# batra-mlp-lab/visdial

Hardware: AMD Instinct MI355X
Metric: QA-rounds/sec training mn-att-ques-im-hist+disc (batch 20x10x100) (higher is better)
Workload: dtype f32 operands and results; the option recurrence multiplies the EXACT 3-way bf16 split of both operands (9 bf16 MFMA products per fp32 product, f32 accumulate: fp32-grade, errors at the f32 MFMA's own level) -- its two step kernels and its weight-gradient contraction; f32 MFMA (v_mfma_f32_32x32x2_f32

## Files before the change

### visdial_amd/csrc/split_core.h

```cpp
#pragma once
#include "gemm_core.h"
#include "paths.h"

typedef __bf16 vd_bf16x8 __attribute__((ext_vector_type(8)));

__device__ __forceinline__ void vd_split3(const float4& u, const float4& w, vd_bf16x8& hi, vd_bf16x8& mid, vd_bf16x8& lo) {
  const float v[8] = {u.x, u.y, u.z, u.w, w.x, w.y, w.z, w.w};
#pragma unroll
  for (int i = 0; i < 8; ++i) {
    const __bf16 h = (__bf16)v[i];
    const float r1 = v[i] - (float)h;
    const __bf16 m = (__bf16)r1;
    const float r2 = r1 - (float)m;
    hi[i] = h; mid[i] = m; lo[i] = (__bf16)r2;
  }
}

static __global__ void __launch_bounds__(256) f32_to_bf16x3_kernel(const float* __restrict__ src, vd_bf16_bits* __restrict__ dst, long n4, long plane) {
  const long i = (long)blockIdx.x * 256 + threadIdx.x;
  if (i >= n4) return;
  const float4 v = reinterpret_cast<const float4*>(src)[i];
  float4 r1, r2;
  typedef __bf16 bf4 __attribute__((ext_vector_type(4)));
  const bf4 h = {(__bf16)v.x, (__bf16)v.y, (__bf16)v.z, (__bf16)v.w};
  r1.x = v.x - (float)h[0]; r1.y = v.y - (float)h[1]; r1.z = v.z - (float)h[2]; r1.w = v.w - (float)h[3];
  const bf4 m = {(__bf16)r1.x, (__bf16)r1.y, (__bf16)r1.z, (__bf16)r1.w};
  r2.x = r1.x - (float)m[0]; r2.y = r1.y - (float)m[1]; r2.z = r1.z - (float)m[2]; r2.w = r1.w - (float)m[3];
  const bf4 l = {(__bf16)r2.x, (__bf16)r2.y, (__bf16)r2.z, (__bf16)r2.w};
  *reinterpret_cast<bf4*>(dst + i * 4) = h;
  *reinterpret_cast<bf4*>(dst + plane + i * 4) = m;
  *reinterpret_cast<bf4*>(dst + 2 * plane + i * 4) = l;
}
static int weights_to_bf16x3(const float* src, vd_bf16_bits* dst, long n, hipStream_t s) {
  hipLaunchKernelGGL(f32_to_bf16x3_kernel, dim3((unsigned)((n / 4 + 255) / 256)), dim3(256), 0, s, src, dst, n / 4, n);
  VD_LAUNCH_CHECK();
  return VD_OK;
}

struct SplitCfg {
    static constexpr int NT = 4, WM = 4, THREADS = 64 * WM;
  static constexpr int BM = 32 * WM, BN = 128, KS = 32;
  static constexpr int BTILE = BN * 64;
  static constexpr int STAGE = 3 * BTILE;
  static constexpr int LDS_BYTES = 2 * STAGE;
  static constexpr int SCR = LDS_BYTES / WM / 4;
  static_assert(SCR >= 32 * QUAD_LD, "quad_to_tile's 32 rows of QUAD_LD floats");
};

#ifndef VD_SPLIT_CG
#define VD_SPLIT_CG 2
#endif
static_assert(VD_SPLIT_CG >= 1 && VD_SPLIT_CG <= 8 && 8 % VD_SPLIT_CG == 0, "the XCD grid is VD_SPLIT_CG x (8 / VD_SPLIT_CG)");
__device__ __forceinline__ bool split_tile_of(int bid, int nwg, int tiles_m, int tiles_n, int& tile_m, int& tile_n) {
  constexpr int CG = VD_SPLIT_CG, RG = 8 / CG;
  if ((tiles_n % CG) == 0 && tiles_n >= 8) {
    const int xcd = bid & 7, li = bid >> 3, cpg = tiles_n / CG, rpg = (tiles_m + RG - 1) / RG;
    tile_n = (xcd % CG) * cpg + li % cpg;
    tile_m = (xcd / CG) * rpg + li / cpg;
    return tile_m < tiles_m && li / cpg < rpg;
  }
  const int wg = xcd_remap(bid, nwg);
  tile_n = wg % tiles_n;
  tile_m = wg / tiles_n;
  return true;
}
__device__ __forceinline__ int split_swz(int q) { return (0x78 >> (2 * (q & 3))) & 3; }
static int split_grid(int tiles_m, int tiles_n) {
  constexpr int CG = VD_SPLIT_CG, RG = 8 / CG;
  if ((tiles_n % CG) == 0 && tiles_n >= 8) return 8 * ((tiles_m + RG - 1) / RG) * (tiles_n / CG);
  return tiles_m * tiles_n;
}

template <int NPROD, class Epi>
__global__ void __launch_bounds__(SplitCfg::THREADS, 3)
gemm_split_kernel(int M, int N, int K, int tiles_n, const float* A, long lda, const vd_bf16_bits* B, long ldb, long bplane, Epi epi) {
  using Cfg = SplitCfg;
  constexpr int NT = Cfg::NT;
  extern __shared__ __attribute__((aligned(16))) float smem[];
  int tile_m, tile_n;
  if (!split_tile_of((int)blockIdx.x, (int)gridDim.x, (M + Cfg::BM - 1) / Cfg::BM, tiles_n, tile_m, tile_n)) return;
  const int row_base = tile_m * Cfg::BM, col_base = tile_n * Cfg::BN;
  constexpr int NIB = 24 / Cfg::WM;
  const int tid = (int)threadIdx.x, lane = tid & 63;
  const int wm = __builtin_amdgcn_readfirstlane(tid >> 6);
  const int nfull = K / 32, nm = nfull + ((K >> 4) & 1);
  const int wrow = row_base + wm * 32;
  const int g = lane >> 4, l15 = lane & 15;

  vd_f32x4 acc[2][2 * NT];
#pragma unroll
  for (int rt = 0; rt < 2; ++rt)
#pragma unroll
    for (int j = 0; j < 2 * NT; ++j)
#pragma unroll
      for (int r = 0; r < 4; ++r) acc[rt][j][r] = 0.f;

  typename EpiPreOf<Epi>::type pre;
  if constexpr (EpiPreOf<Epi>::value) epi.preload(pre, wrow, lane, M);

  unsigned aoff[2];
#pragma unroll
  for (int rt = 0; rt < 2; ++rt) aoff[rt] = (unsigned)(((long)min(wrow + rt * 16 + l15, M - 1) * lda + g * 8) * 4);
  float4 an[2][2];
  auto load_a = [&](int m) {
    const char* ak = reinterpret_cast<const char*>(A + (long)m * 32);
    const bool live = m < nfull || g < 2;
#pragma unroll
    for (int rt = 0; rt < 2; ++rt) {
      an[rt][0] = an[rt][1] = make_float4(0.f, 0.f, 0.f, 0.f);
      if (live) {
        an[rt][0] = *reinterpret_cast<const float4*>(ak + aoff[rt]);
        an[rt][1] = *reinterpret_cast<const float4*>(ak + aoff[rt] + 16);
      }
    }
  };
  const int csrc = (lane & 3) ^ split_swz(lane >> 4);
  unsigned voffb[NIB];
#pragma unroll
  for (int i = 0; i < NIB; ++i) {
    const int r = ((wm * NIB + i) & 7) * 16 + (lane >> 2);
    voffb[i] = (unsigned)(((long)min(col_base + r, N - 1) * ldb + csrc * 8) * 2);
  }
  const unsigned lds0 = (unsigned)(uintptr_t)smem;
  auto issue_b = [&](int m, int st) {
    const unsigned back = m < nfull ? 0u : (unsigned)(csrc >> 1) * 32u;
#pragma unroll
    for (int i = 0; i < NIB; ++i) {
      const int q = wm * NIB + i;
      glds16(voffb[i] - back, reinterpret_cast<const float*>(B + (long)(q >> 3) * bplane + (long)m * 32), lds0 + st * Cfg::STAGE + q * 1024);
    }
  };
  const int bfrag = l15 * 64 + ((g ^ split_swz(l15 >> 2)) * 16);

  if (nm > 0) {
    issue_b(0, 0);
    load_a(0);
    int st = 0;
    for (int m = 0; m < nm; ++m) {
      vd_bf16x8 ap[2][3];
#pragma unroll
      for (int rt = 0; rt < 2; ++rt) vd_split3(an[rt][0], an[rt][1], ap[rt][0], ap[rt][1], ap[rt][2]);
      asm volatile("s_waitcnt vmcnt(0)" ::: "memory");
      asm volatile("s_barrier" ::: "memory");
      if (m + 1 < nm) {
        issue_b(m + 1, st ^ 1);
        load_a(m + 1);
      }
      const char* sbase = reinterpret_cast<const char*>(smem) + st * Cfg::STAGE + bfrag;
#pragma unroll
      for (int p = 2; p >= 0; --p) {
        vd_bf16x8 bp[2 * NT];
#pragma unroll
        for (int j = 0; j < 2 * NT; ++j) {
          const vd_f32x4 t = *reinterpret_cast<const vd_f32x4*>(sbase + p * Cfg::BTILE + j * 1024);
          bp[j] = __builtin_bit_cast(vd_bf16x8, t);
        }
#pragma unroll
        for (int i = 2; i >= 0; --i) {
          constexpr int LIM = NPROD >= 9 ? 4 : NPROD >= 6 ? 2 : NPROD >= 3 ? 1 : 0;
          if (i + p > LIM) continue;
#pragma unroll
          for (int rt = 0; rt < 2; ++rt)
#pragma unroll
            for (int j = 0; j < 2 * NT; ++j) acc[rt][j] = __builtin_amdgcn_mfma_f32_16x16x32_bf16(ap[rt][i], bp[j], acc[rt][j], 0, 0, 0);
        }
      }
      asm volatile("s_waitcnt lgkmcnt(0)\n\ts_barrier" ::: "memory");
      st ^= 1;
    }
  }
  float* scr = smem + wm * Cfg::SCR;
  f32x16 tile[NT];
#pragma unroll
  for (int j = 0; j < NT; ++j) tile[j] = quad_to_tile(acc[0][2 * j], acc[0][2 * j + 1], acc[1][2 * j], acc[1][2 * j + 1], scr, lane);
  if constexpr (EpiPreOf<Epi>::value) epi(tile, wrow, col_base, lane, M, N, scr, &pre);
  else epi(tile, wrow, col_base, lane, M, N, scr);
}

template <int NPROD, class Epi>
static int launch_gemm_split(int M, int N, int K, const float* A, long lda, const vd_bf16_bits* B, long ldb, long bplane, const Epi& e,
                             hipStream_t stream) {
  if (M <= 0 || N <= 0) return VD_OK;
  using Cfg = SplitCfg;
  VD_CHECK_ARG(K % 16 == 0 && lda % 4 == 0 && ldb % 8 == 0 && (long)M * lda * 4 < (1L << 32) && (long)N * ldb * 2 < (1L << 32),
               "launch_gemm_split: unsupported shape M=%d N=%d K=%d", M, N, K);
  const int tiles_m = vd_cdiv(M, Cfg::BM), tiles_n = vd_cdiv(N, Cfg::BN);
  auto kern = gemm_split_kernel<NPROD, Epi>;
  static bool attr_set = false;
  if (!attr_set) {
    VD_HIP(hipFuncSetAttribute(reinterpret_cast<const void*>(kern), hipFuncAttributeMaxDynamicSharedMemorySize, 160 * 1024));
    attr_set = true;
  }
  hipLaunchKernelGGL(kern, dim3(split_grid(tiles_m, tiles_n)), dim3(Cfg::THREADS), Cfg::LDS_BYTES, stream, M, N, K, tiles_n, A, lda, B, ldb, bplane, e);
  VD_LAUNCH_CHECK();
  return VD_OK;
}

template <class Epi>
static int launch_gemm_split(int nprod, int M, int N, int K, const float* A, long lda, const vd_bf16_bits* B, long ldb, long bplane,
                             const Epi& e, hipStream_t stream) {
  if (nprod == 9) return launch_gemm_split<9>(M, N, K, A, lda, B, ldb, bplane, e, stream);
  if (nprod == 6) return launch_gemm_split<6>(M, N, K, A, lda, B, ldb, bplane, e, stream);
  return launch_gemm_split<3>(M, N, K, A, lda, B, ldb, bplane, e, stream);
}

struct SplitTnCfg {
  static constexpr int BM = 256, BN = 128, THREADS = 256;
  static constexpr int ATILE = 16 * BM * 4;
  static constexpr int BTILE = 16 * BN * 4;
  static constexpr int STAGE = ATILE + BTILE;
  static constexpr int LDS_BYTES = 2 * STAGE;
};
static_assert(SplitTnCfg::BM == VD_SPLIT_TN_BM && SplitTnCfg::BN == VD_SPLIT_TN_BN, "paths.h vd_tn_split_tiles");

template <int NPROD>
__global__ void __launch_bounds__(256, 2)
gemm_split_tn_kernel(int M, int N, int kchunk, int K, int tiles, int tiles_n, int splits, const float* A, long lda, const float* B, long ldb,
                     float* C, long ldc) {
  using Cfg = SplitTnCfg;
  extern __shared__ __attribute__((aligned(16))) float smem[];
  int tile, split;
  if ((splits & 7) == 0) {
    const int xcd = (int)blockIdx.x & 7, li = (int)blockIdx.x >> 3;
    split = xcd * (splits >> 3) + li / tiles;
    tile = li % tiles;
  } else {
    split = (int)blockIdx.x / tiles;
    tile = (int)blockIdx.x % tiles;
  }
  const int m_base = (tile / tiles_n) * Cfg::BM, n_base = (tile % tiles_n) * Cfg::BN;
  const int ks = split * kchunk, ke = min(K, ks + kchunk);
  const int nm = ke > ks ? (ke - ks) / 16 : 0;
  const int tid = (int)threadIdx.x, lane = tid & 63;
  const int wm = __builtin_amdgcn_readfirstlane(tid >> 6);

  f32x16 acc[2][4];
#pragma unroll
  for (int mb = 0; mb < 2; ++mb)
#pragma unroll
    for (int j = 0; j < 4; ++j)
#pragma unroll
      for (int r = 0; r < 16; ++r) acc[mb][j][r] = 0.f;

  unsigned voffa[4], voffb[2];
#pragma unroll
  for (int i = 0; i < 4; ++i) voffa[i] = (unsigned)(((long)(wm * 4 + i) * lda + m_base + lane * 4) * 4);
#pragma unroll
  for (int i = 0; i < 2; ++i) voffb[i] = (unsigned)(((long)((wm * 2 + i) * 2 + (lane >> 5)) * ldb + n_base + (lane & 31) * 4) * 4);
  const unsigned lds0 = (unsigned)(uintptr_t)smem;
  auto issue = [&](int m, int st) {
    const unsigned base = lds0 + st * Cfg::STAGE;
    const float* ak = A + (long)(ks + m * 16) * lda;
    const float* bk = B + (long)(ks + m * 16) * ldb;
#pragma unroll
    for (int i = 0; i < 2; ++i) glds16(voffb[i], bk, base + Cfg::ATILE + (wm * 2 + i) * 1024);
#pragma unroll
    for (int i = 0; i < 4; ++i) glds16(voffa[i], ak, base + (wm * 4 + i) * 1024);
  };
  const int hi = lane >> 5, l31 = lane & 31;

  if (nm > 0) {
    issue(0, 0);
    int st = 0;
    for (int m = 0; m < nm; ++m) {
      if (m + 1 < nm) {
        issue(m + 1, st ^ 1);
        asm volatile("s_waitcnt vmcnt(6)" ::: "memory");
      } else {
        asm volatile("s_waitcnt vmcnt(0)" ::: "memory");
      }
      asm volatile("s_barrier" ::: "memory");
      const float* sA = reinterpret_cast<const float*>(reinterpret_cast<const char*>(smem) + st * Cfg::STAGE) + (hi * 8) * Cfg::BM + wm * 64 + l31;
      const float* sB = reinterpret_cast<const float*>(reinterpret_cast<const char*>(smem) + st * Cfg::STAGE + Cfg::ATILE) + (hi * 8) * Cfg::BN + l31;
      vd_bf16x8 ap[2][3], bp[2][3];
      auto load_b = [&](int j, vd_bf16x8 (&dst)[3]) {
        const float* p = sB + j * 32;
        const float4 u = make_float4(p[0], p[Cfg::BN], p[2 * Cfg::BN], p[3 * Cfg::BN]);
        const float4 w = make_float4(p[4 * Cfg::BN], p[5 * Cfg::BN], p[6 * Cfg::BN], p[7 * Cfg::BN]);
        vd_split3(u, w, dst[0], dst[1], dst[2]);
      };
#pragma unroll
      for (int mb = 0; mb < 2; ++mb) {
        const float* p = sA + mb * 32;
        const float4 u = make_float4(p[0], p[Cfg::BM], p[2 * Cfg::BM], p[3 * Cfg::BM]);
        const float4 w = make_float4(p[4 * Cfg::BM], p[5 * Cfg::BM], p[6 * Cfg::BM], p[7 * Cfg::BM]);
        vd_split3(u, w, ap[mb][0], ap[mb][1], ap[mb][2]);
      }
      load_b(0, bp[0]);
#pragma unroll
      for (int j = 0; j < 4; ++j) {
        __builtin_amdgcn_sched_barrier(0);
        if (j + 1 < 4) load_b(j + 1, bp[(j + 1) & 1]);
#pragma unroll
        for (int pb = 2; pb >= 0; --pb)
#pragma unroll
          for (int pa = 2; pa >= 0; --pa) {
            constexpr int LIM = NPROD >= 9 ? 4 : NPROD >= 6 ? 2 : NPROD >= 3 ? 1 : 0;
            if (pa + pb > LIM) continue;
#pragma unroll
            for (int mb = 0; mb < 2; ++mb) acc[mb][j] = __builtin_amdgcn_mfma_f32_32x32x16_bf16(ap[mb][pa], bp[j & 1][pb], acc[mb][j], 0, 0, 0);
          }
        if (j + 1 < 4) {
          __builtin_amdgcn_sched_group_barrier(0x100, 4, 0);
#pragma unroll
          for (int i = 0; i < 18; ++i) {
            __builtin_amdgcn_sched_group_barrier(0x008, 1, 0);
            __builtin_amdgcn_sched_group_barrier(0x002, 4, 0);
          }
        }
      }
      asm volatile("s_waitcnt lgkmcnt(0)\n\ts_barrier" ::: "memory");
      st ^= 1;
    }
  }
  if (nm == 0) return;
  const EpiAtomic<4> e{C, ldc};
#pragma unroll
  for (int mb = 0; mb < 2; ++mb) e(acc[mb], m_base + wm * 64 + mb * 32, n_base, lane, M, N);
}

template <int NPROD>
static int launch_gemm_split_tn(int M, int N, int K, const float* A, long lda, const float* B, long ldb, float* C, long ldc, hipStream_t stream) {
  using Cfg = SplitTnCfg;
  VD_CHECK_ARG(M % Cfg::BM == 0 && N % Cfg::BN == 0 && K % 16 == 0 && lda % 4 == 0 && ldb % 4 == 0 && 16L * lda * 4 < (1L << 31) && 16L * ldb * 4 < (1L << 31),
               "launch_gemm_split_tn: unsupported shape M=%d N=%d K=%d", M, N, K);
  if (K == 0) return VD_OK;
  const int tiles_n = N / Cfg::BN, tiles = (M / Cfg::BM) * tiles_n;
  int splits = vd_cdiv(2L * vd_num_cus(), tiles);
  splits = (splits + 7) & ~7;
  int kchunk = vd_cdiv(vd_cdiv(K, splits), 16) * 16;
  if (kchunk < 64) kchunk = 64;
  splits = vd_cdiv(K, kchunk);
  if (splits >= 8) splits = (splits + 7) & ~7;
  auto kern = gemm_split_tn_kernel<NPROD>;
  static bool attr_set = false;
  if (!attr_set) {
    VD_HIP(hipFuncSetAttribute(reinterpret_cast<const void*>(kern), hipFuncAttributeMaxDynamicSharedMemorySize, 160 * 1024));
    attr_set = true;
  }
  hipLaunchKernelGGL(kern, dim3(tiles * splits), dim3(256), Cfg::LDS_BYTES, stream, M, N, kchunk, K, tiles, tiles_n, splits, A, lda, B, ldb, C, ldc);
  VD_LAUNCH_CHECK();
  return VD_OK;
}
```

Measured before the change: 9222.

## Tighten split-GEMM inner loops: packed bf16 split, peeled full-tile steps, unrolled stages

Replaces the scalar fp32-to-3xbf16 split with packed v_cvt_pk_bf16_f32 plus bit-mask widening, cutting VALU work per split. The step GEMM kernel now peels full K-tiles into a specialized step that skips the tail-clamping offset logic, and halves the B-fragment register batch to reduce VGPR pressure. The TN weight-gradient kernel unrolls the double-buffer loop by two so stage offsets become compile-time constants. These changes add code size and rely on inline asm that the compiler cannot schedule around freely.

Measured after the change: 9411, median of 6. 2.1% higher.

```diff
diff --git a/visdial_amd/csrc/split_core.h b/visdial_amd/csrc/split_core.h
--- a/visdial_amd/csrc/split_core.h
+++ b/visdial_amd/csrc/split_core.h
@@ -4,16 +4,43 @@
 
 typedef __bf16 vd_bf16x8 __attribute__((ext_vector_type(8)));
 
+__device__ __forceinline__ unsigned vd_cvt_pk_bf16(float a, float b) {
+  unsigned r;
+  asm("v_cvt_pk_bf16_f32 %0, %1, %2" : "=v"(r) : "v"(a), "v"(b));
+  return r;
+}
+__device__ __forceinline__ float vd_bf16_lo_f32(unsigned p) {
+  float r;
+  asm("v_lshlrev_b32 %0, 16, %1" : "=v"(r) : "v"(p));
+  return r;
+}
+__device__ __forceinline__ float vd_bf16_hi_f32(unsigned p) {
+  float r;
+  asm("v_and_b32 %0, 0xffff0000, %1" : "=v"(r) : "v"(p));
+  return r;
+}
+__device__ __forceinline__ float vd_sub_f32(float a, float b) {
+  float r;
+  asm("v_sub_f32 %0, %1, %2" : "=v"(r) : "v"(a), "v"(b));
+  return r;
+}
+__device__ __forceinline__ void vd_split3_pair(float a, float b, unsigned& hi, unsigned& mid, unsigned& lo) {
+  hi = vd_cvt_pk_bf16(a, b);
+  const float ra = vd_sub_f32(a, vd_bf16_lo_f32(hi)), rb = vd_sub_f32(b, vd_bf16_hi_f32(hi));
+  mid = vd_cvt_pk_bf16(ra, rb);
+  lo = vd_cvt_pk_bf16(vd_sub_f32(ra, vd_bf16_lo_f32(mid)), vd_sub_f32(rb, vd_bf16_hi_f32(mid)));
+}
+
+typedef unsigned vd_u32x4 __attribute__((ext_vector_type(4)));
 __device__ __forceinline__ void vd_split3(const float4& u, const float4& w, vd_bf16x8& hi, vd_bf16x8& mid, vd_bf16x8& lo) {
-  const float v[8] = {u.x, u.y, u.z, u.w, w.x, w.y, w.z, w.w};
-#pragma unroll
-  for (int i = 0; i < 8; ++i) {
-    const __bf16 h = (__bf16)v[i];
-    const float r1 = v[i] - (float)h;
-    const __bf16 m = (__bf16)r1;
-    const float r2 = r1 - (float)m;
-    hi[i] = h; mid[i] = m; lo[i] = (__bf16)r2;
-  }
+  unsigned h[4], m[4], l[4];
+  vd_split3_pair(u.x, u.y, h[0], m[0], l[0]);
+  vd_split3_pair(u.z, u.w, h[1], m[1], l[1]);
+  vd_split3_pair(w.x, w.y, h[2], m[2], l[2]);
+  vd_split3_pair(w.z, w.w, h[3], m[3], l[3]);
+  hi = __builtin_bit_cast(vd_bf16x8, (vd_u32x4){h[0], h[1], h[2], h[3]});
+  mid = __builtin_bit_cast(vd_bf16x8, (vd_u32x4){m[0], m[1], m[2], m[3]});
+  lo = __builtin_bit_cast(vd_bf16x8, (vd_u32x4){l[0], l[1], l[2], l[3]});
 }
 
 static __global__ void __launch_bounds__(256) f32_to_bf16x3_kernel(const float* __restrict__ src, vd_bf16_bits* __restrict__ dst, long n4, long plane) {
@@ -132,41 +159,69 @@
   };
   const int bfrag = l15 * 64 + ((g ^ split_swz(l15 >> 2)) * 16);
 
+  auto load_a_full = [&](int m) {
+    const char* ak = reinterpret_cast<const char*>(A + (long)m * 32);
+#pragma unroll
+    for (int rt = 0; rt < 2; ++rt) {
+      an[rt][0] = *reinterpret_cast<const float4*>(ak + aoff[rt]);
+      an[rt][1] = *reinterpret_cast<const float4*>(ak + aoff[rt] + 16);
+    }
+  };
+  auto issue_b_full = [&](int m, int st) {
+#pragma unroll
+    for (int i = 0; i < NIB; ++i) {
+      const int q = wm * NIB + i;
+      glds16(voffb[i], reinterpret_cast<const float*>(B + (long)(q >> 3) * bplane + (long)m * 32), lds0 + st * Cfg::STAGE + q * 1024);
+    }
+  };
+
+  auto step = [&](int m, int st, auto full_next) {
+    vd_bf16x8 ap[2][3];
+#pragma unroll
+    for (int rt = 0; rt < 2; ++rt) vd_split3(an[rt][0], an[rt][1], ap[rt][0], ap[rt][1], ap[rt][2]);
+    __builtin_amdgcn_sched_barrier(0);
+    asm volatile("s_waitcnt vmcnt(0)" ::: "memory");
+    asm volatile("s_barrier" ::: "memory");
+    if constexpr (decltype(full_next)::value) {
+      issue_b_full(m + 1, st ^ 1);
+      load_a_full(m + 1);
+    } else if (m + 1 < nm) {
+      issue_b(m + 1, st ^ 1);
+      load_a(m + 1);
+    }
+    __builtin_amdgcn_sched_barrier(0);
+    const char* sbase = reinterpret_cast<const char*>(smem) + st * Cfg::STAGE + bfrag;
+#pragma unroll
+    for (int p = 2; p >= 0; --p)
+#pragma unroll
+      for (int jh = 0; jh < 2; ++jh) {
+        vd_bf16x8 bp[NT];
+#pragma unroll
+        for (int j = 0; j < NT; ++j) {
+          const vd_f32x4 t = *reinterpret_cast<const vd_f32x4*>(sbase + p * Cfg::BTILE + (jh * NT + j) * 1024);
+          bp[j] = __builtin_bit_cast(vd_bf16x8, t);
+        }
+#pragma unroll
+        for (int i = 2; i >= 0; --i) {
+          constexpr int LIM = NPROD >= 9 ? 4 : NPROD >= 6 ? 2 : NPROD >= 3 ? 1 : 0;
+          if (i + p > LIM) continue;
+#pragma unroll
+          for (int rt = 0; rt < 2; ++rt)
+#pragma unroll
+            for (int j = 0; j < NT; ++j)
+              acc[rt][jh * NT + j] = __builtin_amdgcn_mfma_f32_16x16x32_bf16(ap[rt][i], bp[j], acc[rt][jh * NT + j], 0, 0, 0);
+        }
+      }
+    asm volatile("s_waitcnt lgkmcnt(0)\n\ts_barrier" ::: "memory");
+  };
   if (nm > 0) {
     issue_b(0, 0);
     load_a(0);
-    int st = 0;
-    for (int m = 0; m < nm; ++m) {
-      vd_bf16x8 ap[2][3];
-#pragma unroll
-      for (int rt = 0; rt < 2; ++rt) vd_split3(an[rt][0], an[rt][1], ap[rt][0], ap[rt][1], ap[rt][2]);
-      asm volatile("s_waitcnt vmcnt(0)" ::: "memory");
-      asm volatile("s_barrier" ::: "memory");
-      if (m + 1 < nm) {
-        issue_b(m + 1, st ^ 1);
-        load_a(m + 1);
-      }
-      const char* sbase = reinterpret_cast<const char*>(smem) + st * Cfg::STAGE + bfrag;
-#pragma unroll
-      for (int p = 2; p >= 0; --p) {
-        vd_bf16x8 bp[2 * NT];
-#pragma unroll
-        for (int j = 0; j < 2 * NT; ++j) {
-          const vd_f32x4 t = *reinterpret_cast<const vd_f32x4*>(sbase + p * Cfg::BTILE + j * 1024);
-          bp[j] = __builtin_bit_cast(vd_bf16x8, t);
-        }
-#pragma unroll
-        for (int i = 2; i >= 0; --i) {
-          constexpr int LIM = NPROD >= 9 ? 4 : NPROD >= 6 ? 2 : NPROD >= 3 ? 1 : 0;
-          if (i + p > LIM) continue;
-#pragma unroll
-          for (int rt = 0; rt < 2; ++rt)
-#pragma unroll
-            for (int j = 0; j < 2 * NT; ++j) acc[rt][j] = __builtin_amdgcn_mfma_f32_16x16x32_bf16(ap[rt][i], bp[j], acc[rt][j], 0, 0, 0);
-        }
-      }
-      asm volatile("s_waitcnt lgkmcnt(0)\n\ts_barrier" ::: "memory");
-      st ^= 1;
+    int m = 0;
+    for (; m + 1 < nfull; ++m) step(m, m & 1, std::true_type{});
+    if (m < nm) {
+      step(m, m & 1, std::false_type{});
+      if (++m < nm) step(m, m & 1, std::false_type{});
     }
   }
   float* scr = smem + wm * Cfg::SCR;
@@ -259,59 +314,68 @@
   };
   const int hi = lane >> 5, l31 = lane & 31;
 
+  int mb1 = 32;
+  asm("" : "+v"(mb1));
+  const float* sA0 = smem + (hi * 8) * Cfg::BM + wm * 64 + l31;
+  const float* sA1 = sA0 + mb1;
+  const float* sB0 = smem + Cfg::ATILE / 4 + (hi * 8) * Cfg::BN + l31;
+  auto step = [&](int m, auto stage) {
+    constexpr int st = decltype(stage)::value;
+    if (m + 1 < nm) {
+      issue(m + 1, st ^ 1);
+      asm volatile("s_waitcnt vmcnt(6)" ::: "memory");
+    } else {
+      asm volatile("s_waitcnt vmcnt(0)" ::: "memory");
+    }
+    asm volatile("s_barrier" ::: "memory");
+    const float* sB = sB0 + st * (Cfg::STAGE / 4);
+    vd_bf16x8 ap[2][3], bp[2][3];
+    auto load_b = [&](int j, vd_bf16x8 (&dst)[3]) {
+      const float* p = sB + j * 32;
+      const float4 u = make_float4(p[0], p[Cfg::BN], p[2 * Cfg::BN], p[3 * Cfg::BN]);
+      const float4 w = make_float4(p[4 * Cfg::BN], p[5 * Cfg::BN], p[6 * Cfg::BN], p[7 * Cfg::BN]);
+      vd_split3(u, w, dst[0], dst[1], dst[2]);
+    };
+#pragma unroll
+    for (int mb = 0; mb < 2; ++mb) {
+      const float* p = (mb ? sA1 : sA0) + st * (Cfg::STAGE / 4);
+      const float4 u = make_float4(p[0], p[Cfg::BM], p[2 * Cfg::BM], p[3 * Cfg::BM]);
+      const float4 w = make_float4(p[4 * Cfg::BM], p[5 * Cfg::BM], p[6 * Cfg::BM], p[7 * Cfg::BM]);
+      vd_split3(u, w, ap[mb][0], ap[mb][1], ap[mb][2]);
+    }
+    load_b(0, bp[0]);
+#pragma unroll
+    for (int j = 0; j < 4; ++j) {
+      __builtin_amdgcn_sched_barrier(0);
+      if (j + 1 < 4) load_b(j + 1, bp[(j + 1) & 1]);
+#pragma unroll
+      for (int pb = 2; pb >= 0; --pb)
+#pragma unroll
+        for (int pa = 2; pa >= 0; --pa) {
+          constexpr int LIM = NPROD >= 9 ? 4 : NPROD >= 6 ? 2 : NPROD >= 3 ? 1 : 0;
+          if (pa + pb > LIM) continue;
+#pragma unroll
+          for (int mb = 0; mb < 2; ++mb) acc[mb][j] = __builtin_amdgcn_mfma_f32_32x32x16_bf16(ap[mb][pa], bp[j & 1][pb], acc[mb][j], 0, 0, 0);
+        }
+      if (j + 1 < 4) {
+        __builtin_amdgcn_sched_group_barrier(0x100, 4, 0);
+#pragma unroll
+        for (int i = 0; i < 18; ++i) {
+          __builtin_amdgcn_sched_group_barrier(0x008, 1, 0);
+          __builtin_amdgcn_sched_group_barrier(0x002, 4, 0);
+        }
+      }
+    }
+    asm volatile("s_waitcnt lgkmcnt(0)\n\ts_barrier" ::: "memory");
+  };
   if (nm > 0) {
     issue(0, 0);
-    int st = 0;
-    for (int m = 0; m < nm; ++m) {
-      if (m + 1 < nm) {
-        issue(m + 1, st ^ 1);
-        asm volatile("s_waitcnt vmcnt(6)" ::: "memory");
-      } else {
-        asm volatile("s_waitcnt vmcnt(0)" ::: "memory");
-      }
-      asm volatile("s_barrier" ::: "memory");
-      const float* sA = reinterpret_cast<const float*>(reinterpret_cast<const char*>(smem) + st * Cfg::STAGE) + (hi * 8) * Cfg::BM + wm * 64 + l31;
-      const float* sB = reinterpret_cast<const float*>(reinterpret_cast<const char*>(smem) + st * Cfg::STAGE + Cfg::ATILE) + (hi * 8) * Cfg::BN + l31;
-      vd_bf16x8 ap[2][3], bp[2][3];
-      auto load_b = [&](int j, vd_bf16x8 (&dst)[3]) {
-        const float* p = sB + j * 32;
-        const float4 u = make_float4(p[0], p[Cfg::BN], p[2 * Cfg::BN], p[3 * Cfg::BN]);
-        const float4 w = make_float4(p[4 * Cfg::BN], p[5 * Cfg::BN], p[6 * Cfg::BN], p[7 * Cfg::BN]);
-        vd_split3(u, w, dst[0], dst[1], dst[2]);
-      };
-#pragma unroll
-      for (int mb = 0; mb < 2; ++mb) {
-        const float* p = sA + mb * 32;
-        const float4 u = make_float4(p[0], p[Cfg::BM], p[2 * Cfg::BM], p[3 * Cfg::BM]);
-        const float4 w = make_float4(p[4 * Cfg::BM], p[5 * Cfg::BM], p[6 * Cfg::BM], p[7 * Cfg::BM]);
-        vd_split3(u, w, ap[mb][0], ap[mb][1], ap[mb][2]);
-      }
-      load_b(0, bp[0]);
-#pragma unroll
-      for (int j = 0; j < 4; ++j) {
-        __builtin_amdgcn_sched_barrier(0);
-        if (j + 1 < 4) load_b(j + 1, bp[(j + 1) & 1]);
-#pragma unroll
-        for (int pb = 2; pb >= 0; --pb)
-#pragma unroll
-          for (int pa = 2; pa >= 0; --pa) {
-            constexpr int LIM = NPROD >= 9 ? 4 : NPROD >= 6 ? 2 : NPROD >= 3 ? 1 : 0;
-            if (pa + pb > LIM) continue;
-#pragma unroll
-            for (int mb = 0; mb < 2; ++mb) acc[mb][j] = __builtin_amdgcn_mfma_f32_32x32x16_bf16(ap[mb][pa], bp[j & 1][pb], acc[mb][j], 0, 0, 0);
-          }
-        if (j + 1 < 4) {
-          __builtin_amdgcn_sched_group_barrier(0x100, 4, 0);
-#pragma unroll
-          for (int i = 0; i < 18; ++i) {
-            __builtin_amdgcn_sched_group_barrier(0x008, 1, 0);
-            __builtin_amdgcn_sched_group_barrier(0x002, 4, 0);
-          }
-        }
-      }
-      asm volatile("s_waitcnt lgkmcnt(0)\n\ts_barrier" ::: "memory");
-      st ^= 1;
-    }
+    int m = 0;
+    for (; m + 1 < nm; m += 2) {
+      step(m, std::integral_constant<int, 0>{});
+      step(m + 1, std::integral_constant<int, 1>{});
+    }
+    if (m < nm) step(m, std::integral_constant<int, 0>{});
   }
   if (nm == 0) return;
   const EpiAtomic<4> e{C, ldc};
```
